# vidify/old-audiosync

Hardware: AMD Instinct MI355X
Metric: cross-correlations/sec (N=1440000 float32 pairs) (higher is better)
Workload: dtype f32; 1 GPU; batched xcorr, N=1440000 frames/sample (source 2N), 124 pairs per GPU per step, 48 kHz mono float32, planted delays, SNR 0 dB; sample_len=1440000, pairs_per_gpu=124, group=124, split=600x2400x16, layout=real-column, parallelism=pairs sharded over 1 GPU(s), one process per GPU, RCCL all_gather of results

## Files before the change

include/audiosync/xcorr_hip.h:

```cpp
#ifndef AUDIOSYNC_XCORR_HIP_H
#define AUDIOSYNC_XCORR_HIP_H

#include <stddef.h>
#include <stdint.h>

#ifdef __cplusplus
extern "C" {
#endif

typedef struct asx_plan asx_plan;


int asx_device_count(void);
int asx_current_device(void);
const char *asx_last_error(void);
int asx_abi_version(void);


asx_plan *asx_plan_create(size_t sample_len, size_t max_batch, int device);
asx_plan *asx_plan_create_ex(size_t sample_len, size_t max_batch, int device, const char *split);
int asx_plan_placement(asx_plan *plan, double ms[2], int *kept);
void asx_plan_destroy(asx_plan *plan);

int asx_plan_peak_overflows(asx_plan *plan, uint64_t *count);
int asx_plan_peak_repairs(asx_plan *plan, uint64_t *count);
int asx_plan_set_exact(asx_plan *plan, int on);
size_t asx_plan_peak_capacity(const asx_plan *plan);

int asx_plan_set_lag_window(asx_plan *plan, int64_t lag_min, int64_t lag_max);
int asx_plan_lag_window(const asx_plan *plan, int64_t *lag_min, int64_t *lag_max);

int asx_plan_set_pearson(asx_plan *plan, int spectral);
int asx_plan_pearson_modes(asx_plan *plan, uint64_t counts[3]);

int asx_plan_set_prune(asx_plan *plan, int on);
int asx_plan_prune_stats(asx_plan *plan, uint64_t *tiles_transformed, uint64_t *tiles_total);

int asx_plan_set_qstore(asx_plan *plan, int mode);
int asx_plan_qstore_stats(asx_plan *plan, uint64_t out[4]);

size_t asx_plan_sample_len(const asx_plan *plan);
size_t asx_plan_fft_len(const asx_plan *plan);
int asx_plan_split(const asx_plan *plan, int *m1, int *m2, int *tile_cols);
int asx_plan_layout(const asx_plan *plan);
int asx_plan_threads(const asx_plan *plan, int *threads_cols, int *threads_rows);
size_t asx_plan_group(const asx_plan *plan);
size_t asx_plan_workspace_bytes(const asx_plan *plan);


int asx_xcorr_f64(asx_plan *plan, const double *source, const double *sample, long *lag,
                  double *coefficient);
int asx_plan_narrowed_calls(asx_plan *plan, uint64_t *count);

int asx_xcorr_batch_f32(asx_plan *plan, const float *source, const float *sample, size_t batch,
// ... 214 lines not shown
```

old-audiosync_amd/__init__.py:

```python
from .hipxcorr import (
    LIB_PATH, AsxError, Plan, Stream, abi_version, device_count, lib, pearson_f64, planmath_candidates, planmath_describe, planmath_group_form, planmath_kernel_table, planmath_kernels,
    planmath_table, planmath_twiddles, band_bins, results_to_ms_dev, synth_pairs_dev, topk_best_dev, xcorr_batch_multi,
    Comm, PinnedArray, result_bytes, shard_range, closure_args, pool_closure, pool_closure_dev, phat_topk_args, pool_phat_topk_args,
)
```

old-audiosync_amd/csrc/asx_api.hip:

```cpp
#include "audiosync/xcorr_hip.h"

#include "asx_internal.h"
#include "dev_mem.h"
#include "plan_math.h"
#include "shard_driver.h"
#include "host_narrow.h"

#include <algorithm>
#include <cassert>
#include <cmath>
#include <cstdarg>
#include <cstdio>
#include <cstdlib>
#include <cstring>
#include <dlfcn.h>
#include <mutex>
#include <string>
#include <thread>
#include <type_traits>
#include <vector>

static thread_local std::string g_err;

static int fail(const char *fmt, ...)
// ... 112 lines not shown
    uint32_t *over_list = nullptr, *over_n = nullptr;
    volatile uint32_t *h_over_n = nullptr;
    size_t over_cap = 0;
    std::vector<uint32_t> h_over;
    unsigned long long repaired = 0;
    bool exact = true;
    int64_t win_lo = 0, win_hi = 0;
    bool spectral = false;
    unsigned long long *mode_count = nullptr;
    bool prunable = false;
    bool prune = false;
    unsigned long long *prune_stats = nullptr;
    int qstore = 1;
    unsigned long long *qstore_stats = nullptr;
    uint64_t qstore_redone = 0;
    bool tune_placement = false, placement_done = false;
    double placement_ms[2] = { 0.0, 0.0 };
    int placement_kept = -1;
    struct Staging {
        float *src = nullptr, *smp = nullptr;
        int64_t *lag = nullptr; double *coef = nullptr; int32_t *ret = nullptr;
    } st;
    struct Staging64 { double *src = nullptr, *smp = nullptr; } st64;
    float *pin32 = nullptr;
    unsigned long long narrowed = 0;

    bool profiling = false;
    size_t prof_depth = 1, prof_calls = 0, prof_ring = 0;
    std::vector<std::vector<hipEvent_t>> evr;
    std::vector<size_t> prof_groups;
// ... 135 lines not shown
        *p->h_over_n = 0;
        HIP_TRY(hipHostGetDevicePointer(&dptr, h, 0));
        d_over_host = (uint32_t *)dptr;
    }
    for (int l = 0; l < p->nlanes; l++) {
        p->lanes[l].pk.over_list = p->over_list;
        p->lanes[l].pk.over_n = p->over_n;
        p->lanes[l].pk.over_host = d_over_host;
        p->lanes[l].pk.over_cap = (uint32_t)p->over_cap;
    }
    p->spectral = d.rlayout != 0;
    if (const char *e = getenv("ASX_PEARSON")) p->spectral = p->spectral && strcmp(e, "direct") != 0;
    p->prune = p->prunable;
    if (const char *e = getenv("ASX_PRUNE")) p->prune = p->prune && atoi(e) != 0;
    if (const char *e = getenv("ASX_QSTORE")) p->qstore = std::min(2, std::max(0, atoi(e)));
    if (const char *e = getenv("ASX_EXACT")) p->exact = atoi(e) != 0;
    p->win_lo = -(int64_t)p->host.N;
    p->win_hi = (int64_t)p->host.N - 1;
    HIP_TRY(hipEventCreateWithFlags(&p->fork, hipEventDisableTiming));
    d.stamps = nullptr;
    d.stamp_kernel = 0;
    if (const char *e = getenv("ASX_STAMPS")) {
        unsigned long long *st = nullptr;
        p->stamp_blocks = g * (size_t)std::max(h.M1 + 1, 2 * h.ntiles);
        if (dev_alloc(m, &st, p->stamp_blocks * 8)) return -1;
        HIP_TRY(hipMemset(st, 0, p->stamp_blocks * 8 * sizeof(unsigned long long)));
        d.stamps = st;
        d.stamp_kernel = !strcmp(e, "fwd") ? 1 : !strcmp(e, "inv") ? 2 : 0;
    }
    {
// ... 205 lines not shown
    HIP_TRY(hipMemcpy(v, p->prune_stats, sizeof v, hipMemcpyDeviceToHost));
    *tiles_transformed = v[0];
    *tiles_total = v[1];
    return 0;
}

extern "C" int asx_plan_set_qstore(asx_plan *p, int mode)
{
    if (!p) return fail("asx_plan_set_qstore: null argument");
    if (mode < 0 || mode > 2) return fail("asx_plan_set_qstore: mode %d (0 off, 1 auto, 2 always)", mode);
    std::lock_guard<std::mutex> guard(p->lock);
    p->qstore = mode;
    return 0;
}

extern "C" int asx_plan_qstore_stats(asx_plan *p, uint64_t out[4])
{
    if (!p || !out) return fail("asx_plan_qstore_stats: null argument");
    PlanCall c(p);
    if (!c.dg.ok) return fail("cannot select device %d", p->device);
    out[0] = out[1] = out[2] = out[3] = 0;
    if (!p->qstore_stats) return 0;
    HIP_TRY(hipDeviceSynchronize());
    unsigned long long v[4];
    HIP_TRY(hipMemcpy(v, p->qstore_stats, sizeof v, hipMemcpyDeviceToHost));
    out[0] = v[0]; out[1] = v[1]; out[2] = p->qstore_redone; out[3] = v[3];
    return 0;
}

extern "C" int asx_plan_peak_repairs(asx_plan *p, uint64_t *count)
// ... 250 lines not shown
    const AsxGroupForm form = asx_group_form(
        { .rlayout = P.rlayout != 0, .plan_prune = p->prune, .plan_spectral = p->spectral, .band_sums = pk.band != nullptr,
          .over_list = pk.over_list != nullptr, .f32_inputs = std::is_same<TIn, float>::value, .f32_abi = o.f32_abi, .listed = o.listed,
          .r_out = o.r_out != nullptr, .own_lists = o.pk != nullptr, .k = o.topk.k, .search = call.kind, .weight = o.weight,
          .pool = x.pool != nullptr, .bc = x.bc, .qstore = o.qstore });
    const AsxPeakWs fin = form.appends ? pk : asx_peak_unlisted(pk);
    const AsxPeakWs tk = form.tail == ASX_TAIL_SPECTRAL ? pk : asx_peak_unbanded(pk);
    const AsxPoolPair *pl = x.pool ? W.pool : nullptr;
    const AsxSpectra &from = pl ? p->bank.c : p->bslot;
    const AsxSpectra C{ (pl || (x.bc & 1)) ? from.cx : W.zxa, (pl || (x.bc & 2)) ? from.cy : W.zya, pk.nrm_part, tk.band, form.bc, pl };
    AsxPrune U = W.prune;
    U.q_rows = form.qstore ? asx_qstore_rows(P, (int)g, p->qstore) : 0;
    U.q_row_a = P.M1 / 3;
    U.pair_base = o.pair_base;
    if (!U.q_rows) { U.list = nullptr; U.redo = nullptr; }
    if (mark(0)) return -1;
    if (form.fwd == ASX_FWD_POOL) {
        const AsxPoolArgs A{ x.pool->rows, (uint64_t)x.first, (uint64_t)x.pool->nsrc, (uint64_t)x.pool->nsmp, (uint64_t)x.src_step,
                             (uint64_t)x.smp_step, from.nrm, from.band };
        asx_launch_pool_resolve(P, A, W.pool, C.nrm, C.band, (int)g, s);
    } else if (form.fwd == ASX_FWD_REAL) {
        asx_launch_fwd_cols_r(P, (x.bc & 1) ? nullptr : x.src, x.src_step, (x.bc & 2) ? nullptr : x.smp, x.smp_step, 0, (int)g, C, false, s);
        for (unsigned which = 0; which < 2; which++)
            if (x.bc & (1 << which)) asx_launch_bcast_aux(P, from.nrm, from.band, C.nrm, C.band, (int)g, which, s);
    } else if (x.src_step == 2 * (size_t)P.N && x.smp_step == P.N) {
        asx_launch_fwd_cols(P, x.src, x.smp, W.zxa, W.zya, tk, (int)g, s);
    } else {
        for (size_t k = 0; k < g; k++) {
            AsxPeakWs one = tk;
            one.nrm_part = pk.nrm_part + k * 2 * (size_t)P.ntiles;
// ... 12 lines not shown
    auto search = [&](int j) { return AsxSearch::of(p->win_lo, p->win_hi, P.N, x.win, x.win_step, W.tk, j); };
    const double votes = form.weight == ASX_W_PHAT_BAND ? o.fband.votes(P.N) : (double)P.F;
    auto pass = [&](const AsxSearch &find, bool first) -> int {
        float *const r_out = first ? o.r_out : nullptr;
        if (form.rows == ASX_ROWS_PACKED) asx_launch_inv_cols(P, q, tk, r_out, (int)g, s, find);
        else asx_launch_inv_cols_r(P, q, tk, r_out, (int)g, s, find, form.pruned ? &U : nullptr);
        if (first && mark(3)) return -1;
        if (form.tail == ASX_TAIL_PHAT) {
            asx_launch_phat_finalize(P, fin, W.seg, K > 1 ? nullptr : y.peak, votes, (int)g, s, find);
            if (first && mark(4)) return -1;
            asx_launch_pearson(in, P.N, W.seg, W.psums, out.lag, out.coef, out.ret, (int)g, s);
            if (o.near.frac)
                asx_launch_phat_near(P, q, W.seg, votes, o.near.h, find, pl, o.near.frac, o.near.near, (int)g, s);
            return 0;
        }
        asx_launch_finalize(P, fin, W.seg, (int)g, s, o.pair_base, find);
        asx_launch_refine(P, in, pk, W.seg, (int)g, s, dot_blocks, form.tail == ASX_TAIL_DIRECT, find);
        if (first && mark(4)) return -1;
        if (form.tail == ASX_TAIL_DIRECT)
            asx_launch_pearson(in, P.N, W.seg, W.psums, out.lag, out.coef, out.ret, (int)g, s);
        else if constexpr (std::is_same<TIn, float>::value)
            asx_launch_pearson_spectral_f32(P, in, find, tk, W.spec, W.seg, W.psums, out.lag, out.coef, out.ret, (int)g, s);
        return 0;
    };
    if (pass(call, true)) return -1;
    if (U.q_rows && form.takeback) asx_launch_qstore_takeback(U, W.spec, (int)g, s);
    if (call.kind == AsxSearch::ROWS && K == 1) asx_launch_invalid_rows(call.rows, P.N, y.lag, y.coef, y.ret, (int)g, s);
    if (pl && K == 1) asx_launch_invalid_pairs(pl, y.lag, y.coef, y.ret, y.peak, (int)g, s);
    for (int j = 0; K > 1 && j < K; j++) {
        if (j > 0 && pass(search(j), false)) return -1;
        if (form.tail == ASX_TAIL_PHAT && y.peak) asx_launch_topk_peak(W.tk, pk, call, P.N, (int)g, j, K, votes, y.peak, s);
        asx_launch_topk_step(W.tk, W.seg, pk, call, P.N, (int)g, j, K, o.topk.sep, y.lag, y.coef, y.ret, s);
    }
    if (pl && K > 1) asx_launch_invalid_pairs_k(pl, K, y.lag, y.coef, y.ret, y.peak, (int)g, s);
    if (mark(5)) return -1;
    HIP_TRY(hipGetLastError());
    return 0;
}

template <typename TIn>
static int second_look(asx_plan *p, const Pairs<TIn> &xi, const Results &yi, hipStream_t s, const Topk &topk)
// ... 1392 lines not shown

extern "C" int asx_planmath_group_form(const int *ask, int nask, int *out, int nout)
{
    if (!ask || !out || nask != ASX_GROUP_ASK_INTS || nout != ASX_GROUP_FORM_INTS)
        return fail("asx_planmath_group_form: %d and %d ints, not %d and %d", nask, nout, ASX_GROUP_ASK_INTS, ASX_GROUP_FORM_INTS);
    AsxGroupAsk a;
    a.rlayout = ask[0]; a.plan_prune = ask[1]; a.plan_spectral = ask[2]; a.band_sums = ask[3]; a.over_list = ask[4];
    a.f32_inputs = ask[5]; a.f32_abi = ask[6]; a.listed = ask[7]; a.r_out = ask[8]; a.own_lists = ask[9]; a.k = ask[10];
    a.search = ask[11]; a.weight = (AsxWeight)ask[12]; a.pool = ask[13]; a.bc = ask[14]; a.qstore = ask[15];
    const AsxGroupForm f = asx_group_form(a);
    const int v[ASX_GROUP_FORM_INTS] = { f.fwd, f.rows, f.weight, f.bc, f.pruned, f.tail, f.appends, f.qstore, f.takeback };
    memcpy(out, v, sizeof v);
    return 0;
}

extern "C" int asx_planmath_describe(size_t sample_len, const char *split, uint32_t *F, uint32_t *src_valid,
                                     int *M1, int *M2, int *T, int *nst1, int *radix1, int *nst2,
                                     int *radix2)
{
    AsxHostPlan h;
    std::string err = asx_host_plan_build(sample_len, split, &h);
    if (!err.empty()) return fail("%s", err.c_str());
    *F = h.F; *src_valid = h.src_valid; *M1 = h.M1; *M2 = h.M2; *T = h.T;
    *nst1 = h.st1.nstages; *nst2 = h.st2.nstages;
    for (int i = 0; i < h.st1.nstages; i++) radix1[i] = h.st1.radix[i];
    for (int i = 0; i < h.st2.nstages; i++) radix2[i] = h.st2.radix[i];
    return 0;
}

extern "C" int asx_planmath_candidates(size_t sample_len, size_t max_count, char *out, size_t cap)
// ... 32 lines not shown
```

old-audiosync_amd/csrc/asx_internal.h:

```cpp
#pragma once

#include <hip/hip_runtime.h>
#include <stdint.h>
#include <type_traits>

#define ASX_MAX_STAGES 12
#define ASX_TW_LOG 11
#define ASX_TW_LO (1u << ASX_TW_LOG)
#define ASX_THREADS 256
#define ASX_FFT_THREADS_MAX 512
#define ASX_COL_LOADS 10
#define ASX_ROW_STEPS 5
#define ASX_PEARSON_BLOCKS_MAX 512
#define ASX_DC_STATS_DOUBLES (4 + 2 * 128)
#define ASX_BOUND_C 4.0f
#define ASX_PRUNE_DELTA 6.103515625e-5f
#define ASX_PRUNE_FLOOR_PER_TERM 3.944304526105059e-31
#define ASX_PRUNE_T 16
#define ASX_Q_ALL 0xFFFFFFFFFFFFFFFFull
#define ASX_QSTORE_C 1.75
#define ASX_QSTORE_REDO 0x80000000u
__host__ __device__ inline bool asx_q_stored(unsigned long long w, int tile)
{
    const unsigned t = (unsigned)tile;
// ... 422 lines not shown
void asx_launch_pool_resolve(const AsxDev &P, const AsxPoolArgs &A, AsxPoolPair *out, float *nrm, float2 *band, int npairs,
                             hipStream_t s);
void asx_launch_invalid_pairs(const AsxPoolPair *pl, int64_t *lag, double *coef, int32_t *ret, double *peak, int npairs, hipStream_t s);
void asx_launch_invalid_pairs_k(const AsxPoolPair *pl, int k, int64_t *lag, double *coef, int32_t *ret, double *peak, int npairs,
                                hipStream_t s);
void asx_launch_finalize(const AsxDev &P, const AsxPeakWs &W, AsxSeg *seg, int npairs, hipStream_t s, uint32_t pair_base,
                         const AsxSearch &q);
void asx_launch_topk_step(AsxTopkWs T, const AsxSeg *seg, const AsxPeakWs &W, const AsxSearch &call, uint32_t N, int npairs, int j,
                          int k, int64_t sep, int64_t *lag, double *coef, int32_t *ret, hipStream_t s);
void asx_launch_topk_peak(const AsxTopkWs &T, const AsxPeakWs &W, const AsxSearch &call, uint32_t N, int npairs, int j, int k, double f,
                          double *peak, hipStream_t s);
void asx_launch_invalid_rows(const AsxWinRows &rows, uint32_t N, int64_t *lag, double *coef, int32_t *ret, int npairs, hipStream_t s);
template <typename TIn>
void asx_launch_refine(const AsxDev &P, const AsxInputs<TIn> &in, const AsxPeakWs &W, AsxSeg *seg, int npairs, hipStream_t s,
                       int dot_blocks, bool pick, const AsxSearch &q);
template <typename TIn>
void asx_launch_pearson(const AsxInputs<TIn> &in, uint32_t basis_len, const AsxSeg *seg, double *psums, int64_t *lag, double *coef,
                        int32_t *ret, int npairs, hipStream_t s);
void asx_launch_pearson_partial_spec_f32(const AsxInputs<float> &in, uint32_t basis_len, const AsxSeg *seg, const AsxSpecWs &S,
                                         double *psums, int npairs, hipStream_t s);
void asx_launch_pearson_spectral_f32(const AsxDev &P, const AsxInputs<float> &in, const AsxSearch &q, const AsxPeakWs &W,
                                     const AsxSpecWs &S, AsxSeg *seg, double *psums, int64_t *lag, double *coef, int32_t *ret,
                                     int npairs, hipStream_t s);
int asx_launch_debug_spec_pick(const AsxDev &P, const AsxSpecWs &S, const AsxSeg *seg, size_t pair, double *out, hipStream_t s);
void asx_launch_results_to_ms(const int64_t *lag, const double *coef, const int32_t *ret, size_t batch,
                              double min_confidence, double sample_rate, int64_t *lag_ms, int32_t *accept,
                              hipStream_t s);
void asx_launch_topk_best(const int64_t *lag, const double *coef, const int32_t *ret, size_t batch, int k, int64_t *best_lag,
                          double *best_coef, int32_t *best_ret, int32_t *best_entry, hipStream_t s);
#define ASX_CLOSURE_LAG_LIMIT ((int64_t)1 << 40)
void asx_launch_pool_closure(const int64_t *lag, const double *coef, const int32_t *ret, uint32_t C, int k, int64_t tol,
                             int min_confirm, int root, int32_t *votes, int64_t *best_lag, double *best_coef, int32_t *best_ret,
                             int32_t *best_entry, int32_t *confirm, int32_t *d_root, int64_t *offset, int32_t *support,
                             int32_t *placed, hipStream_t s);
void asx_launch_cvt_f64_f32(const double *in, float *out, size_t n, hipStream_t s);
unsigned asx_pearson_blocks(uint32_t basis_len);
template <typename TIn>
void asx_launch_dc_remove(const TIn *src, const TIn *smp, uint32_t N, double scale, double *stats, float *out, hipStream_t s);
// ... 3 lines not shown
```

old-audiosync_amd/csrc/pearson_spectral.hip:

```cpp
#include "asx_internal.h"
#include "xcorr_dev.h"


static_assert(ASX_PREP_BLOCKS <= ASX_PREP_BLOCKS_MAX, "AsxSpecWs::part is sized for ASX_PREP_BLOCKS_MAX blocks per pair");
#ifndef ASX_PREP_THREADS
#define ASX_PREP_THREADS 1024
#endif

namespace {

struct Acc2 {
    double s1, s2;
};

__device__ __forceinline__ void acc1(Acc2 &a, float f)
{
    const double v = (double)f;
    a.s1 += v;
    a.s2 = fma(v, v, a.s2);
}
__device__ __forceinline__ void acc4(Acc2 &a, float4 v) { acc1(a, v.x); acc1(a, v.y); acc1(a, v.z); acc1(a, v.w); }

template <uint32_t NTP> __device__ __forceinline__ void direct_range(const float *__restrict__ x, uint32_t lo, uint32_t hi, Acc2 &a, uint32_t tid)
{
// ... 120 lines not shown
template <int NTP, int NB> __global__ __launch_bounds__(NTP) void k_pearson_prep_xl(const AsxDev *__restrict__ Pp, const float *__restrict__ src,
                                                                       const float *__restrict__ smp, const AsxPoolPair *__restrict__ PL,
                                                                       AsxPeakWs W, AsxSpecWs S, AsxSeg *__restrict__ seg,
                                                                       const AsxTopkPair *__restrict__ X)
{
    const uint32_t seed = X[blockIdx.y].z.seed;
#define ASX_SRC_OF(pair) PL[pair].src_off
#define ASX_SMP_OF(pair) PL[pair].smp_off
#include "pearson_prep_body.h"
}

__global__ __launch_bounds__(64) void k_pearson_final_spec(const AsxSeg *__restrict__ seg, const double *__restrict__ psums, uint32_t nb,
                                                            AsxSpecWs S, int64_t *__restrict__ lag,
                                                            double *__restrict__ coef, int32_t *__restrict__ ret)
{
    const size_t pair = blockIdx.x;
    const AsxSeg s = seg[pair];
    const AsxSpecPick d = asx_spec_pick(s, S.part + pair * (size_t)(S.nb * 4), S.nb, S.hdr + pair * ASX_SPEC_HDR, S.tol, S.N);
    const int mode = (int)S.hdr[pair * ASX_SPEC_HDR + 3];
    PStat v;
    v.n = v.mx = v.my = v.mxx = v.myy = v.cxy = 0.0;
    if (mode != ASX_PM_FAST) {
        for (uint32_t b = threadIdx.x; b < nb; b += 64u) {
            const double *p = psums + (pair * nb + b) * 6;
            PStat o;
            o.n = p[0];
            if (o.n != 0.0) { o.mx = p[1]; o.my = p[2]; o.mxx = p[3]; o.myy = p[4]; o.cxy = p[5]; v = pstat_merge(v, o); }
        }
        v = pstat_wave_merge(v);
    }
    if (threadIdx.x == 0) {
        double c;
        if (mode == ASX_PM_DIRECT) {
            c = v.cxy / sqrt(v.mxx * v.myy);
        } else {
            const double n = d.n, Sx = d.Sx, Sxx = d.Sxx, Sy = d.Sy, Syy = d.Syy;
            double sxy = d.r;
            if (mode == ASX_PM_CORR) sxy -= v.cxy + v.n * v.mx * v.my;
            c = (sxy - Sx * Sy / n) / sqrt((Sxx - Sx * Sx / n) * (Syy - Sy * Sy / n));
            c = c > 1.0 ? 1.0 : c < -1.0 ? -1.0 : c;
        }
        if (lag) lag[pair] = s.lag;
        coef[pair] = c;
        if (ret) ret[pair] = (s.flags & ASX_SEG_INEXACT) ? 1 : (c != c) ? -1 : 0;
        atomicAdd(S.mode_count + mode, 1ull);
    }
}

template <int NTP, int NB>
static void launch_prep(const AsxDev &P, const AsxInputs<float> &in, const AsxSearch &q, const AsxPeakWs &W, const AsxSpecWs &S,
                        AsxSeg *seg, int npairs, hipStream_t s)
{
    const dim3 grid(NB, npairs), block(NTP);
    if (in.pl && q.kind == AsxSearch::TOPK)
        hipLaunchKernelGGL((k_pearson_prep_xl<NTP, NB>), grid, block, 0, s, P.self_dev, in.src, in.smp, in.pl, W, S, seg, q.tk);
    else if (in.pl && q.kind == AsxSearch::ROWS)
        hipLaunchKernelGGL((k_pearson_prep_pl<NTP, NB>), grid, block, 0, s, P.self_dev, in.src, in.smp, in.pl, W, S, seg, q.rows);
    else if (in.pl)
        hipLaunchKernelGGL((k_pearson_prep_l<NTP, NB>), grid, block, 0, s, P.self_dev, in.src, in.smp, in.pl, W, S, seg, q.seed());
    else if (q.kind == AsxSearch::TOPK)
        hipLaunchKernelGGL((k_pearson_prep_x<NTP, NB>), grid, block, 0, s, P.self_dev, in.src, in.smp, in.src_pitch, in.smp_pitch, W, S,
                           seg, q.tk);
    else if (q.kind == AsxSearch::ROWS)
        hipLaunchKernelGGL((k_pearson_prep_p<NTP, NB>), grid, block, 0, s, P.self_dev, in.src, in.smp, in.src_pitch, in.smp_pitch, W, S,
                           seg, q.rows);
    else
        hipLaunchKernelGGL((k_pearson_prep<NTP, NB>), grid, block, 0, s, P.self_dev, in.src, in.smp, in.src_pitch, in.smp_pitch, W, S,
                           seg, q.seed());
}

static bool prep_long_tracks(const AsxDev &P) { return (size_t)P.band_rows * (size_t)P.M2 >= 16384; }

void asx_launch_pearson_spectral_f32(const AsxDev &P, const AsxInputs<float> &in, const AsxSearch &q, const AsxPeakWs &W,
                                     const AsxSpecWs &S0, AsxSeg *seg, double *psums, int64_t *lag, double *coef, int32_t *ret,
                                     int npairs, hipStream_t s)
{
    AsxSpecWs S = S0;
    S.N = P.N;
    const bool long_tracks = prep_long_tracks(P);
    S.nb = long_tracks ? ASX_PREP_BLOCKS : 1;
    if (long_tracks) launch_prep<ASX_PREP_THREADS, ASX_PREP_BLOCKS>(P, in, q, W, S, seg, npairs, s);
    else launch_prep<256, 1>(P, in, q, W, S, seg, npairs, s);
    asx_launch_pearson_partial_spec_f32(in, P.N, seg, S, psums, npairs, s);
    hipLaunchKernelGGL(k_pearson_final_spec, dim3(npairs), dim3(64), 0, s, seg, psums, asx_pearson_blocks(P.N), S, lag, coef, ret);
}

__global__ __launch_bounds__(64) void k_debug_spec_pick(const AsxSeg *__restrict__ seg, AsxSpecWs S, size_t pair, double *__restrict__ out)
{
    if (threadIdx.x != 0 || blockIdx.x != 0) return;
    const AsxSpecPick d = asx_spec_pick(seg[pair], S.part + pair * (size_t)(S.nb * 4), S.nb, S.hdr + pair * ASX_SPEC_HDR, S.tol, S.N);
    out[0] = (double)d.mode; out[1] = d.n; out[2] = d.Sx; out[3] = d.Sxx; out[4] = d.Sy; out[5] = d.Syy; out[6] = d.r; out[7] = d.bound;
}

int asx_launch_debug_spec_pick(const AsxDev &P, const AsxSpecWs &S0, const AsxSeg *seg, size_t pair, double *out, hipStream_t s)
{
    AsxSpecWs S = S0;
    S.N = P.N;
    S.nb = prep_long_tracks(P) ? ASX_PREP_BLOCKS : 1;
    hipLaunchKernelGGL(k_debug_spec_pick, dim3(1), dim3(1), 0, s, seg, S, pair, out);
// ... 3 lines not shown
```

old-audiosync_amd/csrc/plan_math.cpp:

```cpp
#include <cstring>
#include <cstdlib>
#include <functional>
#include <algorithm>
#include "plan_math.h"
#include "kernel_table.h"

#include <cmath>
#include <cstdio>
#include <cstdlib>

bool asx_is_smooth(uint64_t n)
{
    if (n == 0) return false;
    for (uint64_t p : { 2ull, 3ull, 5ull })
        while (n % p == 0) n /= p;
    return n == 1;
}

uint64_t asx_next_smooth_even(uint64_t n)
{
    n += n & 1ull;
    if (n < 2) n = 2;
    while (!asx_is_smooth(n)) n += 2;
    return n;
// ... 309 lines not shown
    AsxGroupForm f{};
    f.weight = a.weight;
    f.bc = a.bc;
    const bool phat = a.weight != ASX_W_NONE;
    f.appends = a.listed && !phat;
    const bool spectral = a.f32_inputs && a.plan_spectral && a.f32_abi && a.band_sums && !phat;
    f.tail = phat ? ASX_TAIL_PHAT : spectral ? ASX_TAIL_SPECTRAL : ASX_TAIL_DIRECT;
    f.pruned = a.plan_prune && !phat && a.f32_inputs && a.f32_abi && !a.pool && a.bc == 0 && !a.r_out && !a.own_lists && a.k == 1 &&
               a.search == AsxSearch::ALL;
    f.qstore = f.pruned && a.listed && a.qstore && a.over_list;
    f.takeback = f.qstore && spectral;
    f.fwd = a.pool ? ASX_FWD_POOL : a.rlayout ? ASX_FWD_REAL : ASX_FWD_PACKED;
    f.rows = !a.rlayout ? ASX_ROWS_PACKED : f.pruned ? ASX_ROWS_ENERGY : a.pool ? ASX_ROWS_LISTED : ASX_ROWS_PLAIN;
    return f;
}
```

old-audiosync_amd/csrc/plan_math.h:

```cpp
#pragma once

#include "asx_internal.h"

#include <string>
#include <vector>

struct AsxKernelChoice {
    bool rlayout = false;
    int cols = -1, rows = -1;
    int threads_cols = 0, threads_rows = 0;
    int band_rows = 0;
    bool prunable = false;
};

struct AsxHostPlan {
    size_t N = 0;
    uint32_t F = 0, M = 0, src_valid = 0;
    int M1 = 0, M2 = 0, T = 0, logT = 0, ntiles = 0;
    AsxStages st1{}, st2{};
    std::vector<float2> tw1, tw2, tw2s, tw_lo, tw_hi;
    std::vector<int> k1_of_pos1, pos1_of_k1, pos2_of_k2;
    std::vector<int4> row_tasks;
    bool rlayout = false;
    std::vector<int4> col_pairs;
// ... 34 lines not shown
};
enum AsxFwdForm { ASX_FWD_POOL, ASX_FWD_REAL, ASX_FWD_PACKED };
enum AsxTail { ASX_TAIL_PHAT, ASX_TAIL_DIRECT, ASX_TAIL_SPECTRAL };
struct AsxGroupForm {
    AsxFwdForm fwd;
    AsxRowFlavour rows;
    AsxWeight weight;
    int bc;
    bool pruned;
    AsxTail tail;
    bool appends;
    bool qstore;
    bool takeback;
};
AsxGroupForm asx_group_form(const AsxGroupAsk &a);
constexpr int ASX_GROUP_ASK_INTS = 16, ASX_GROUP_FORM_INTS = 9;
```

old-audiosync_amd/csrc/xcorr_kernels.hip:

```cpp
#include "asx_internal.h"
#include "lds_fft.h"
#include "xcorr_dev.h"
#include "kernel_table.h"

#include <algorithm>
#include <math.h>
#include <type_traits>
#include <stdlib.h>

#ifndef ASX_PART
#define ASX_PART 127
#endif
#define ASX_HAS_PART(bit) ((ASX_PART & (bit)) != 0)

#ifdef ASX_STAMPS
#define ASX_STAMP_AT(kernel, block, slot)                                                            \
    do {                                                                                             \
        if (P.stamps && P.stamp_kernel == (kernel) && threadIdx.x == 0)                              \
            P.stamps[(size_t)(block) * 8 + (slot)] = clock64();                                      \
    } while (0)
#else
#define ASX_STAMP_AT(kernel, block, slot) do {} while (0)
#endif
#define ASX_STAMP(slot) ASX_STAMP_AT(0, task, slot)
// ... 970 lines not shown
        __syncthreads();
        if (threadIdx.x == 0) {
            dd_t t;
            t.hi = red[0][0]; t.lo = red[1][0];
            for (int w = 1; w < ASX_THREADS / 64; w++) {
                dd_t o;
                o.hi = red[0][w]; o.lo = red[1][w];
                t = dd_add(t, o);
            }
            W.refine_val[pair * (size_t)W.cap + c] = t.hi + t.lo;
        }
        __syncthreads();
    }
}

template <class Sel>
__global__ __launch_bounds__(ASX_THREADS) void k_refine_pick(const AsxDev *__restrict__ Pp, AsxPeakWs W, AsxSeg *__restrict__ seg,
                                                              Sel sel)
{
    const uint32_t seed = sel.seed_of(blockIdx.x, Pp->N);
    __shared__ double rkey[ASX_THREADS / 64];
    __shared__ uint32_t ridx[ASX_THREADS / 64];
    const size_t pair = blockIdx.x;
    const uint32_t n = W.refine_n[pair];
    if (n < 2u) return;
    double bk = -INFINITY;
    uint32_t bi = 0xFFFFFFFFu;
    for (uint32_t i = threadIdx.x; i < n; i += ASX_THREADS) {
        const uint32_t idx = W.refine_idx[pair * (size_t)W.cap + i];
        const double v = W.refine_val[pair * (size_t)W.cap + i];
// ... 1238 lines not shown
template <typename TIn>
void asx_launch_refine(const AsxDev &P, const AsxInputs<TIn> &in, const AsxPeakWs &W, AsxSeg *seg, int npairs, hipStream_t s,
                       int dot_blocks, bool pick, const AsxSearch &q)
{
    asx_with_inputs(in, [&](auto at) {
        hipLaunchKernelGGL((k_refine_dots<TIn, decltype(at)>), dim3(dot_blocks, npairs), dim3(ASX_THREADS), 0, s, P.self_dev, in.src,
                           in.smp, at, W);
    });
    if (!pick) return;
    const dim3 grid(npairs), block(ASX_THREADS);
    asx_with_selection(q, [&](auto sel) {
        hipLaunchKernelGGL(k_refine_pick<decltype(sel)>, grid, block, 0, s, P.self_dev, W, seg, sel);
    });
}

unsigned asx_pearson_blocks(uint32_t basis_len)
{
    const uint32_t per_block = 16u * 4u * ASX_THREADS;
    uint32_t nb = (basis_len + per_block - 1) / per_block;
    if (nb > ASX_PEARSON_BLOCKS_MAX) nb = ASX_PEARSON_BLOCKS_MAX;
    if (nb < 1) nb = 1;
    return nb;
}

template <typename TIn, bool SPEC>
static void launch_pearson_partial(const AsxInputs<TIn> &in, uint32_t basis_len, const AsxSeg *seg, const AsxSpecWs &S, double *psums,
                                   int npairs, hipStream_t s)
{
    const dim3 grid(asx_pearson_blocks(basis_len), npairs), block(ASX_THREADS);
    asx_with_inputs(in, [&](auto at) {
// ... 169 lines not shown
```

old-audiosync_amd/hipxcorr.py:

```python
import ctypes
import os
import sys

import numpy as np

_HERE = os.path.dirname(os.path.abspath(__file__))
LIB_PATH = os.path.join(_HERE, "libaudiosync_hip.so")
_lib = None

c_f32p = ctypes.POINTER(ctypes.c_float)
c_f64p = ctypes.POINTER(ctypes.c_double)
c_i64p = ctypes.POINTER(ctypes.c_int64)
c_i32p = ctypes.POINTER(ctypes.c_int32)
c_intp = ctypes.POINTER(ctypes.c_int)

_vp, _sz, _int, _i64, _u64, _dbl, _str = (ctypes.c_void_p, ctypes.c_size_t, ctypes.c_int, ctypes.c_int64, ctypes.c_uint64,
                                          ctypes.c_double, ctypes.c_char_p)
_vpp, _szp, _longp = ctypes.POINTER(_vp), ctypes.POINTER(_sz), ctypes.POINTER(ctypes.c_long)
_u32p, _u64p = ctypes.POINTER(ctypes.c_uint32), ctypes.POINTER(ctypes.c_uint64)

_HEADER_SIGNATURES = {
    "asx_device_count": (_int, []),
    "asx_current_device": (_int, []),
    "asx_last_error": (_str, []),
# ... 11 lines not shown
    "asx_plan_layout": (_int, [_vp]),
    "asx_plan_peak_overflows": (_int, [_vp, _u64p]),
    "asx_plan_peak_repairs": (_int, [_vp, _u64p]),
    "asx_plan_narrowed_calls": (_int, [_vp, _u64p]),
    "asx_plan_set_exact": (_int, [_vp, _int]),
    "asx_plan_set_lag_window": (_int, [_vp, _i64, _i64]),
    "asx_plan_lag_window": (_int, [_vp, c_i64p, c_i64p]),
    "asx_stream_set_lag_window": (_int, [_vp, _i64, _i64]),
    "asx_plan_placement": (_int, [_vp, c_f64p, c_intp]),
    "asx_plan_set_pearson": (_int, [_vp, _int]),
    "asx_plan_pearson_modes": (_int, [_vp, _u64p]),
    "asx_plan_set_prune": (_int, [_vp, _int]),
    "asx_plan_prune_stats": (_int, [_vp, _u64p, _u64p]),
    "asx_plan_set_qstore": (_int, [_vp, _int]),
    "asx_plan_qstore_stats": (_int, [_vp, _u64p]),
    "asx_plan_set_profiling": (_int, [_vp, _int]),
    "asx_plan_last_timings_ms": (_int, [_vp, c_f32p]),
    "asx_plan_timings_ms": (_int, [_vp, _int, c_f32p]),
    "asx_xcorr_f64": (_int, [_vp, c_f64p, c_f64p, _longp, c_f64p]),
    "asx_xcorr_batch_f32": (_int, [_vp, c_f32p, c_f32p, _sz, c_i64p, c_f64p, c_i32p]),
    "asx_xcorr_batch_multi": (_int, [_vpp, _int, c_f32p, c_f32p, _sz, c_i64p, c_f64p, c_i32p]),
    "asx_xcorr_batch_f32_dev": (_int, [_vp, _vp, _vp, _sz, _vp, _vp, _vp, _vp]),
    "asx_xcorr_strided_f32_dev": (_int, [_vp, _vp, _sz, _vp, _sz, _sz, _vp, _vp, _vp, _vp]),
    "asx_xcorr_windowed_f32_dev": (_int, [_vp, _vp, _sz, _vp, _sz, _vp, _sz, _sz, _vp, _vp, _vp, _vp]),
    "asx_xcorr_topk_f32_dev": (_int, [_vp, _vp, _sz, _vp, _sz, _vp, _sz, _sz, _int, _i64, _vp, _vp, _vp, _vp]),
    "asx_xcorr_phat_f32_dev": (_int, [_vp, _vp, _sz, _vp, _sz, _vp, _sz, _sz, _vp, _vp, _vp, _vp, _vp]),
    "asx_xcorr_phat_band_f32_dev": (_int, [_vp, _vp, _sz, _vp, _sz, _vp, _sz, _sz, _i64, _i64, _vp, _vp, _vp, _vp, _vp]),
    "asx_xcorr_phat_sub_f32_dev": (_int, [_vp, _vp, _sz, _vp, _sz, _vp, _sz, _sz, _i64, _i64, _int, _vp, _vp, _vp, _vp, _vp, _vp, _vp]),
    "asx_xcorr_phat_topk_f32_dev": (_int, [_vp, _vp, _sz, _vp, _sz, _vp, _sz, _sz, _i64, _i64, _int, _i64, _vp, _vp, _vp, _vp, _vp]),
    "asx_xcorr_pool_f32_dev": (_int, [_vp, _vp, _sz, _sz, _vp, _sz, _sz, _vp, _vp, _sz, _sz, _vp, _vp, _vp, _vp]),
# ... 36 lines not shown
    "asx_host_malloc": (_vp, [_sz]),
    "asx_host_free": (_int, [_vp]),
    "asx_memcpy_h2d": (_int, [_vp, _vp, _sz]),
    "asx_memcpy_d2h": (_int, [_vp, _vp, _sz]),
    "asx_stream_sync": (_int, [_vp, _vp]),
}

_DIAGNOSTIC_SIGNATURES = {
    "asx_planmath_describe": (_int, [_sz, _str, _u32p, _u32p, c_intp, c_intp, c_intp, c_intp, c_intp, c_intp, c_intp]),
    "asx_planmath_table": (_int, [_sz, _str, _int, c_intp, _sz]),
    "asx_planmath_twiddles": (_int, [_sz, _str, _int, c_f32p, _sz]),
    "asx_planmath_candidates": (_int, [_sz, _sz, _str, _sz]),
    "asx_planmath_kernels": (_int, [_sz, _str, c_intp, c_intp, c_intp]),
    "asx_planmath_kernel_table": (_int, [_int, _int, c_intp]),
    "asx_planmath_group_form": (_int, [c_intp, _int, c_intp, _int]),
    "asx_plan_debug_kernels": (_int, [_vp, c_intp, c_intp, c_intp]),
    "asx_plan_debug_bank": (_int, [_vp, _u64p, _u64p, _u64p]),
    "asx_plan_debug_prune": (_int, [_vp, _sz, c_f32p, c_intp, _sz]),
    "asx_plan_debug_peak": (_int, [_vp, _sz, c_f32p, _u32p, _u32p, _u64p, _vp, _vp, _sz]),
    "asx_plan_debug_spectral": (_int, [_vp, _sz, c_intp, _vp, _sz, c_f64p, ctypes.POINTER(ctypes.c_longlong), c_f64p]),
    "asx_plan_debug_over_list": (_int, [_vp, _u32p, _u32p]),
    "asx_plan_debug_stamps": (ctypes.c_long, [_vp, _vp, _sz]),
}

SIGNATURES = {**_HEADER_SIGNATURES, **_DIAGNOSTIC_SIGNATURES}

ABI_SYMBOLS = list(_HEADER_SIGNATURES)

TOPK_MAX = 8
NEAR_MAX = 8
# ... 114 lines not shown
GROUP_ASK = ("rlayout", "plan_prune", "plan_spectral", "band_sums", "over_list", "f32_inputs", "f32_abi", "listed", "r_out",
             "own_lists", "k", "search", "weight", "pool", "bc", "qstore")
GROUP_FORM = ("fwd", "rows", "weight", "bc", "pruned", "tail", "appends", "qstore", "takeback")
GROUP_ENUMS = {"search": ("all", "window", "rows", "topk"), "weight": ("none", "phat", "phat-band"),
               "fwd": ("pool", "real-column", "packed"), "rows": ("packed", "plain", "energy", "listed"),
               "tail": ("phat", "direct", "spectral")}


def planmath_group_form(**ask):
    if set(ask) != set(GROUP_ASK):
        raise ValueError("planmath_group_form: the ask is %s" % (GROUP_ASK,))
    a = (ctypes.c_int * len(GROUP_ASK))(*(GROUP_ENUMS[n].index(ask[n]) if n in GROUP_ENUMS else int(ask[n]) for n in GROUP_ASK))
    out = (ctypes.c_int * len(GROUP_FORM))()
    _check(lib().asx_planmath_group_form(a, len(a), out, len(out)))
    return {n: GROUP_ENUMS[n][v] if n in GROUP_ENUMS else v if n == "bc" else bool(v) for n, v in zip(GROUP_FORM, out)}


def planmath_candidates(sample_len, max_count=16):
    buf = ctypes.create_string_buffer(64 * max_count + 1)
    n = lib().asx_planmath_candidates(sample_len, max_count, buf, len(buf))
    if n < 0:
        raise AsxError(_err())
    return [x for x in buf.value.decode().split("\n") if x]


def planmath_table(sample_len, which, split=None):
    d = planmath_describe(sample_len, split)
    cap = max(d["M1"], d["M2"])
    buf = (ctypes.c_int * cap)()
    n = lib().asx_planmath_table(sample_len, _split_arg(split), which, buf, cap)
# ... 526 lines not shown

    def pearson_modes(self):
        c = (ctypes.c_uint64 * 3)()
        _check(lib().asx_plan_pearson_modes(self._h, c))
        return tuple(int(v) for v in c)

    def set_prune(self, on=True):
        _check(lib().asx_plan_set_prune(self._h, 1 if on else 0))

    def prune_stats(self):
        return _counters(lib().asx_plan_prune_stats, self._h, 2)

    def set_qstore(self, mode=1):
        _check(lib().asx_plan_set_qstore(self._h, int(mode)))

    def qstore_stats(self):
        c = (ctypes.c_uint64 * 4)()
        _check(lib().asx_plan_qstore_stats(self._h, c))
        return tuple(int(v) for v in c)

    def narrowed_calls(self):
        return _counters(lib().asx_plan_narrowed_calls, self._h, 1)[0]

    def peak_repairs(self):
        return _counters(lib().asx_plan_peak_repairs, self._h, 1)[0]

    @property
    def workspace_bytes(self):
        return lib().asx_plan_workspace_bytes(self._h)

# ... 412 lines not shown
```

Before: 63380 cross-correlations/s.

## Fuse finalize with refine dot products and skip qstore takeback pass

```diff
diff --git a/include/audiosync/xcorr_hip.h b/include/audiosync/xcorr_hip.h
--- a/include/audiosync/xcorr_hip.h
+++ b/include/audiosync/xcorr_hip.h
@@ -38,6 +38,8 @@
 
 int asx_plan_set_qstore(asx_plan *plan, int mode);
 int asx_plan_qstore_stats(asx_plan *plan, uint64_t out[4]);
+
+int asx_plan_set_tail(asx_plan *plan, int on);
 
 size_t asx_plan_sample_len(const asx_plan *plan);
 size_t asx_plan_fft_len(const asx_plan *plan);
diff --git a/old-audiosync_amd/__init__.py b/old-audiosync_amd/__init__.py
--- a/old-audiosync_amd/__init__.py
+++ b/old-audiosync_amd/__init__.py
@@ -1,5 +1,5 @@
 from .hipxcorr import (
-    LIB_PATH, AsxError, Plan, Stream, abi_version, device_count, lib, pearson_f64, planmath_candidates, planmath_describe, planmath_group_form, planmath_kernel_table, planmath_kernels,
+    LIB_PATH, AsxError, Plan, Stream, abi_version, device_count, lib, pearson_f64, planmath_candidates, planmath_describe, planmath_group_form, planmath_group_tail, planmath_kernel_table, planmath_kernels,
     planmath_table, planmath_twiddles, band_bins, results_to_ms_dev, synth_pairs_dev, topk_best_dev, xcorr_batch_multi,
     Comm, PinnedArray, result_bytes, shard_range, closure_args, pool_closure, pool_closure_dev, phat_topk_args, pool_phat_topk_args,
 )
diff --git a/old-audiosync_amd/csrc/asx_api.hip b/old-audiosync_amd/csrc/asx_api.hip
--- a/old-audiosync_amd/csrc/asx_api.hip
+++ b/old-audiosync_amd/csrc/asx_api.hip
@@ -150,6 +150,7 @@
     int qstore = 1;
     unsigned long long *qstore_stats = nullptr;
     uint64_t qstore_redone = 0;
+    bool tail = true;
     bool tune_placement = false, placement_done = false;
     double placement_ms[2] = { 0.0, 0.0 };
     int placement_kept = -1;
@@ -315,6 +316,7 @@
     p->prune = p->prunable;
     if (const char *e = getenv("ASX_PRUNE")) p->prune = p->prune && atoi(e) != 0;
     if (const char *e = getenv("ASX_QSTORE")) p->qstore = std::min(2, std::max(0, atoi(e)));
+    if (const char *e = getenv("ASX_TAIL")) p->tail = atoi(e) != 0;
     if (const char *e = getenv("ASX_EXACT")) p->exact = atoi(e) != 0;
     p->win_lo = -(int64_t)p->host.N;
     p->win_hi = (int64_t)p->host.N - 1;
@@ -550,6 +552,14 @@
     return 0;
 }
 
+extern "C" int asx_plan_set_tail(asx_plan *p, int on)
+{
+    if (!p) return fail("asx_plan_set_tail: null argument");
+    std::lock_guard<std::mutex> guard(p->lock);
+    p->tail = on != 0;
+    return 0;
+}
+
 extern "C" int asx_plan_qstore_stats(asx_plan *p, uint64_t out[4])
 {
     if (!p || !out) return fail("asx_plan_qstore_stats: null argument");
@@ -830,6 +840,7 @@
     U.q_row_a = P.M1 / 3;
     U.pair_base = o.pair_base;
     if (!U.q_rows) { U.list = nullptr; U.redo = nullptr; }
+    const bool short_tail = asx_group_tail_short(form, U.q_rows, p->tail);
     if (mark(0)) return -1;
     if (form.fwd == ASX_FWD_POOL) {
         const AsxPoolArgs A{ x.pool->rows, (uint64_t)x.first, (uint64_t)x.pool->nsrc, (uint64_t)x.pool->nsmp, (uint64_t)x.src_step,
@@ -872,17 +883,23 @@
                 asx_launch_phat_near(P, q, W.seg, votes, o.near.h, find, pl, o.near.frac, o.near.near, (int)g, s);
             return 0;
         }
-        asx_launch_finalize(P, fin, W.seg, (int)g, s, o.pair_base, find);
-        asx_launch_refine(P, in, pk, W.seg, (int)g, s, dot_blocks, form.tail == ASX_TAIL_DIRECT, find);
+        bool fused = false;
+        if constexpr (std::is_same<TIn, float>::value)
+            fused = short_tail && asx_launch_finalize_dots_f32(P, in, fin, W.seg, (int)g, s, dot_blocks, o.pair_base, find);
+        if (!fused) {
+            asx_launch_finalize(P, fin, W.seg, (int)g, s, o.pair_base, find);
+            asx_launch_refine(P, in, pk, W.seg, (int)g, s, dot_blocks, form.tail == ASX_TAIL_DIRECT, find);
+        }
         if (first && mark(4)) return -1;
         if (form.tail == ASX_TAIL_DIRECT)
             asx_launch_pearson(in, P.N, W.seg, W.psums, out.lag, out.coef, out.ret, (int)g, s);
         else if constexpr (std::is_same<TIn, float>::value)
-            asx_launch_pearson_spectral_f32(P, in, find, tk, W.spec, W.seg, W.psums, out.lag, out.coef, out.ret, (int)g, s);
+            asx_launch_pearson_spectral_f32(P, in, find, tk, W.spec, W.seg, W.psums, out.lag, out.coef, out.ret, (int)g, s,
+                                            short_tail ? U.redo : nullptr);
         return 0;
     };
     if (pass(call, true)) return -1;
-    if (U.q_rows && form.takeback) asx_launch_qstore_takeback(U, W.spec, (int)g, s);
+    if (U.q_rows && form.takeback && !short_tail) asx_launch_qstore_takeback(U, W.spec, (int)g, s);
     if (call.kind == AsxSearch::ROWS && K == 1) asx_launch_invalid_rows(call.rows, P.N, y.lag, y.coef, y.ret, (int)g, s);
     if (pl && K == 1) asx_launch_invalid_pairs(pl, y.lag, y.coef, y.ret, y.peak, (int)g, s);
     for (int j = 0; K > 1 && j < K; j++) {
@@ -2305,6 +2322,15 @@
     return 0;
 }
 
+extern "C" int asx_planmath_group_tail(const int *ask, int nask, int q_rows, int plan_tail)
+{
+    int form[ASX_GROUP_FORM_INTS];
+    if (asx_planmath_group_form(ask, nask, form, ASX_GROUP_FORM_INTS)) return -1;
+    AsxGroupForm f{};
+    f.qstore = form[7]; f.takeback = form[8];
+    return asx_group_tail_short(f, q_rows, plan_tail != 0) ? 1 : 0;
+}
+
 extern "C" int asx_planmath_describe(size_t sample_len, const char *split, uint32_t *F, uint32_t *src_valid,
                                      int *M1, int *M2, int *T, int *nst1, int *radix1, int *nst2,
                                      int *radix2)
diff --git a/old-audiosync_amd/csrc/asx_internal.h b/old-audiosync_amd/csrc/asx_internal.h
--- a/old-audiosync_amd/csrc/asx_internal.h
+++ b/old-audiosync_amd/csrc/asx_internal.h
@@ -460,6 +460,8 @@
 template <typename TIn>
 void asx_launch_refine(const AsxDev &P, const AsxInputs<TIn> &in, const AsxPeakWs &W, AsxSeg *seg, int npairs, hipStream_t s,
                        int dot_blocks, bool pick, const AsxSearch &q);
+bool asx_launch_finalize_dots_f32(const AsxDev &P, const AsxInputs<float> &in, const AsxPeakWs &W, AsxSeg *seg, int npairs, hipStream_t s,
+                                  int dot_blocks, uint32_t pair_base, const AsxSearch &q);
 template <typename TIn>
 void asx_launch_pearson(const AsxInputs<TIn> &in, uint32_t basis_len, const AsxSeg *seg, double *psums, int64_t *lag, double *coef,
                         int32_t *ret, int npairs, hipStream_t s);
@@ -467,7 +469,7 @@
                                          double *psums, int npairs, hipStream_t s);
 void asx_launch_pearson_spectral_f32(const AsxDev &P, const AsxInputs<float> &in, const AsxSearch &q, const AsxPeakWs &W,
                                      const AsxSpecWs &S, AsxSeg *seg, double *psums, int64_t *lag, double *coef, int32_t *ret,
-                                     int npairs, hipStream_t s);
+                                     int npairs, hipStream_t s, const unsigned char *voided = nullptr);
 int asx_launch_debug_spec_pick(const AsxDev &P, const AsxSpecWs &S, const AsxSeg *seg, size_t pair, double *out, hipStream_t s);
 void asx_launch_results_to_ms(const int64_t *lag, const double *coef, const int32_t *ret, size_t batch,
                               double min_confidence, double sample_rate, int64_t *lag_ms, int32_t *accept,
diff --git a/old-audiosync_amd/csrc/pearson_final_body.h b/old-audiosync_amd/csrc/pearson_final_body.h
--- /dev/null
+++ b/old-audiosync_amd/csrc/pearson_final_body.h
@@ -0,0 +1,31 @@
+    const size_t pair = blockIdx.x;
+    const AsxSeg s = seg[pair];
+    const AsxSpecPick d = asx_spec_pick(s, S.part + pair * (size_t)(S.nb * 4), S.nb, S.hdr + pair * ASX_SPEC_HDR, S.tol, S.N);
+    const int mode = (int)S.hdr[pair * ASX_SPEC_HDR + 3];
+    PStat v;
+    v.n = v.mx = v.my = v.mxx = v.myy = v.cxy = 0.0;
+    if (mode != ASX_PM_FAST) {
+        for (uint32_t b = threadIdx.x; b < nb; b += 64u) {
+            const double *p = psums + (pair * nb + b) * 6;
+            PStat o;
+            o.n = p[0];
+            if (o.n != 0.0) { o.mx = p[1]; o.my = p[2]; o.mxx = p[3]; o.myy = p[4]; o.cxy = p[5]; v = pstat_merge(v, o); }
+        }
+        v = pstat_wave_merge(v);
+    }
+    if (threadIdx.x == 0) {
+        double c;
+        if (mode == ASX_PM_DIRECT) {
+            c = v.cxy / sqrt(v.mxx * v.myy);
+        } else {
+            const double n = d.n, Sx = d.Sx, Sxx = d.Sxx, Sy = d.Sy, Syy = d.Syy;
+            double sxy = d.r;
+            if (mode == ASX_PM_CORR) sxy -= v.cxy + v.n * v.mx * v.my;
+            c = (sxy - Sx * Sy / n) / sqrt((Sxx - Sx * Sx / n) * (Syy - Sy * Sy / n));
+            c = c > 1.0 ? 1.0 : c < -1.0 ? -1.0 : c;
+        }
+        if (lag) lag[pair] = s.lag;
+        coef[pair] = c;
+        if (ret) ret[pair] = (s.flags & ASX_SEG_INEXACT) ? 1 : (c != c) ? -1 : 0;
+        if (counted) atomicAdd(S.mode_count + mode, 1ull);
+    }
diff --git a/old-audiosync_amd/csrc/pearson_spectral.hip b/old-audiosync_amd/csrc/pearson_spectral.hip
--- a/old-audiosync_amd/csrc/pearson_spectral.hip
+++ b/old-audiosync_amd/csrc/pearson_spectral.hip
@@ -158,37 +158,16 @@
                                                             AsxSpecWs S, int64_t *__restrict__ lag,
                                                             double *__restrict__ coef, int32_t *__restrict__ ret)
 {
-    const size_t pair = blockIdx.x;
-    const AsxSeg s = seg[pair];
-    const AsxSpecPick d = asx_spec_pick(s, S.part + pair * (size_t)(S.nb * 4), S.nb, S.hdr + pair * ASX_SPEC_HDR, S.tol, S.N);
-    const int mode = (int)S.hdr[pair * ASX_SPEC_HDR + 3];
-    PStat v;
-    v.n = v.mx = v.my = v.mxx = v.myy = v.cxy = 0.0;
-    if (mode != ASX_PM_FAST) {
-        for (uint32_t b = threadIdx.x; b < nb; b += 64u) {
-            const double *p = psums + (pair * nb + b) * 6;
-            PStat o;
-            o.n = p[0];
-            if (o.n != 0.0) { o.mx = p[1]; o.my = p[2]; o.mxx = p[3]; o.myy = p[4]; o.cxy = p[5]; v = pstat_merge(v, o); }
-        }
-        v = pstat_wave_merge(v);
-    }
-    if (threadIdx.x == 0) {
-        double c;
-        if (mode == ASX_PM_DIRECT) {
-            c = v.cxy / sqrt(v.mxx * v.myy);
-        } else {
-            const double n = d.n, Sx = d.Sx, Sxx = d.Sxx, Sy = d.Sy, Syy = d.Syy;
-            double sxy = d.r;
-            if (mode == ASX_PM_CORR) sxy -= v.cxy + v.n * v.mx * v.my;
-            c = (sxy - Sx * Sy / n) / sqrt((Sxx - Sx * Sx / n) * (Syy - Sy * Sy / n));
-            c = c > 1.0 ? 1.0 : c < -1.0 ? -1.0 : c;
-        }
-        if (lag) lag[pair] = s.lag;
-        coef[pair] = c;
-        if (ret) ret[pair] = (s.flags & ASX_SEG_INEXACT) ? 1 : (c != c) ? -1 : 0;
-        atomicAdd(S.mode_count + mode, 1ull);
-    }
+    constexpr bool counted = true;
+#include "pearson_final_body.h"
+}
+
+__global__ __launch_bounds__(64) void k_pearson_final_spec_v(const AsxSeg *__restrict__ seg, const double *__restrict__ psums, uint32_t nb,
+                                                              AsxSpecWs S, int64_t *__restrict__ lag, double *__restrict__ coef,
+                                                              int32_t *__restrict__ ret, const unsigned char *__restrict__ redo)
+{
+    const bool counted = !redo[blockIdx.x];
+#include "pearson_final_body.h"
 }
 
 template <int NTP, int NB>
@@ -217,7 +196,7 @@
 
 void asx_launch_pearson_spectral_f32(const AsxDev &P, const AsxInputs<float> &in, const AsxSearch &q, const AsxPeakWs &W,
                                      const AsxSpecWs &S0, AsxSeg *seg, double *psums, int64_t *lag, double *coef, int32_t *ret,
-                                     int npairs, hipStream_t s)
+                                     int npairs, hipStream_t s, const unsigned char *voided)
 {
     AsxSpecWs S = S0;
     S.N = P.N;
@@ -226,7 +205,10 @@
     if (long_tracks) launch_prep<ASX_PREP_THREADS, ASX_PREP_BLOCKS>(P, in, q, W, S, seg, npairs, s);
     else launch_prep<256, 1>(P, in, q, W, S, seg, npairs, s);
     asx_launch_pearson_partial_spec_f32(in, P.N, seg, S, psums, npairs, s);
-    hipLaunchKernelGGL(k_pearson_final_spec, dim3(npairs), dim3(64), 0, s, seg, psums, asx_pearson_blocks(P.N), S, lag, coef, ret);
+    if (voided)
+        hipLaunchKernelGGL(k_pearson_final_spec_v, dim3(npairs), dim3(64), 0, s, seg, psums, asx_pearson_blocks(P.N), S, lag, coef, ret, voided);
+    else
+        hipLaunchKernelGGL(k_pearson_final_spec, dim3(npairs), dim3(64), 0, s, seg, psums, asx_pearson_blocks(P.N), S, lag, coef, ret);
 }
 
 __global__ __launch_bounds__(64) void k_debug_spec_pick(const AsxSeg *__restrict__ seg, AsxSpecWs S, size_t pair, double *__restrict__ out)
diff --git a/old-audiosync_amd/csrc/plan_math.cpp b/old-audiosync_amd/csrc/plan_math.cpp
--- a/old-audiosync_amd/csrc/plan_math.cpp
+++ b/old-audiosync_amd/csrc/plan_math.cpp
@@ -347,3 +347,8 @@
     f.rows = !a.rlayout ? ASX_ROWS_PACKED : f.pruned ? ASX_ROWS_ENERGY : a.pool ? ASX_ROWS_LISTED : ASX_ROWS_PLAIN;
     return f;
 }
+
+bool asx_group_tail_short(const AsxGroupForm &f, int q_rows, bool plan_tail)
+{
+    return plan_tail && f.qstore && f.takeback && q_rows > 0;
+}
diff --git a/old-audiosync_amd/csrc/plan_math.h b/old-audiosync_amd/csrc/plan_math.h
--- a/old-audiosync_amd/csrc/plan_math.h
+++ b/old-audiosync_amd/csrc/plan_math.h
@@ -72,4 +72,5 @@
     bool takeback;
 };
 AsxGroupForm asx_group_form(const AsxGroupAsk &a);
+bool asx_group_tail_short(const AsxGroupForm &f, int q_rows, bool plan_tail);
 constexpr int ASX_GROUP_ASK_INTS = 16, ASX_GROUP_FORM_INTS = 9;
diff --git a/old-audiosync_amd/csrc/xcorr_kernels.hip b/old-audiosync_amd/csrc/xcorr_kernels.hip
--- a/old-audiosync_amd/csrc/xcorr_kernels.hip
+++ b/old-audiosync_amd/csrc/xcorr_kernels.hip
@@ -1008,6 +1008,118 @@
     }
 }
 
+template <typename TIn>
+__device__ __forceinline__ void refine_dot(const TIn *__restrict__ x, const TIn *__restrict__ y, uint32_t N, uint32_t k,
+                                           double (*red)[ASX_THREADS / 64], double *__restrict__ dst)
+{
+    const uint32_t L = 2u * N;
+    const int lane = threadIdx.x & 63, wave = threadIdx.x >> 6;
+    double hi = 0.0, lo = 0.0;
+    for (uint32_t n = threadIdx.x; n < N; n += ASX_THREADS) {
+        uint32_t i = n + k;
+        if (i >= L) i -= L;
+        const double a = (double)x[i], b = (double)y[n];
+        const double p = a * b;
+        double pe = 0.0;
+        if (sizeof(TIn) == sizeof(double)) pe = fma(a, b, -p);
+        const double s = hi + p;
+        const double bb = s - hi;
+        lo += ((hi - (s - bb)) + (p - bb)) + pe;
+        hi = s;
+    }
+    dd_t acc;
+    acc.hi = hi; acc.lo = lo;
+#pragma unroll
+    for (int off = 32; off > 0; off >>= 1) {
+        dd_t o;
+        o.hi = __shfl_xor(acc.hi, off, 64);
+        o.lo = __shfl_xor(acc.lo, off, 64);
+        acc = dd_add(acc, o);
+    }
+    if (lane == 0) { red[0][wave] = acc.hi; red[1][wave] = acc.lo; }
+    __syncthreads();
+    if (threadIdx.x == 0) {
+        dd_t t;
+        t.hi = red[0][0]; t.lo = red[1][0];
+        for (int w = 1; w < ASX_THREADS / 64; w++) {
+            dd_t o;
+            o.hi = red[0][w]; o.lo = red[1][w];
+            t = dd_add(t, o);
+        }
+        *dst = t.hi + t.lo;
+    }
+    __syncthreads();
+}
+
+constexpr int FD_OWN = ASX_CAND_MAX / 8;
+template <typename TIn, class Where>
+__global__ __launch_bounds__(ASX_THREADS) void k_finalize_dots(const AsxDev *__restrict__ Pp, const TIn *__restrict__ src,
+                                                                const TIn *__restrict__ smp, Where at, AsxPeakWs W,
+                                                                AsxSeg *__restrict__ seg, uint32_t pair_base, uint32_t seed)
+{
+    __shared__ double red[2][ASX_THREADS / 64];
+    __shared__ uint32_t own[FD_OWN];
+    __shared__ uint32_t wcount[ASX_THREADS / 64];
+    const size_t pair = blockIdx.x;
+    const uint32_t bx = blockIdx.y, nbx = gridDim.y;
+    const bool writer = bx == 0;
+    const uint32_t ntot = W.cand_n[pair];
+    if (!writer && bx >= ntot) return;
+    const uint32_t N = Pp->N;
+    const int lane = threadIdx.x & 63, wave = threadIdx.x >> 6;
+    const asx_peak_t best = W.pairmax[pair];
+    const bool over = ntot > W.cap;
+    const uint32_t n = (over || ntot < 2u) ? 0u : ntot;
+    uint32_t nsel = 0;
+    if (n) {
+        const float thr = near_max_threshold(peak_key(best), W.bound2[pair]);
+        const AsxCand *c = W.cand + pair * (size_t)W.cap;
+        uint32_t *out = W.refine_idx + pair * (size_t)W.cap;
+        for (uint32_t i0 = 0; i0 < n; i0 += ASX_THREADS) {
+            const uint32_t i = i0 + threadIdx.x;
+            AsxCand e{ 0u, 0.f };
+            if (i < n) e = c[i];
+            const bool keep = i < n && e.key >= thr;
+            const unsigned long long m = __ballot(keep);
+            if (lane == 0) wcount[wave] = (uint32_t)__popcll(m);
+            __syncthreads();
+            uint32_t at_c = nsel + (uint32_t)__popcll(m & ((1ull << lane) - 1ull)), all = 0;
+            for (int w = 0; w < ASX_THREADS / 64; w++) {
+                at_c += w < wave ? wcount[w] : 0u;
+                all += wcount[w];
+            }
+            if (keep) {
+                if (writer) out[at_c] = e.idx;
+                if (at_c % nbx == bx) own[at_c / nbx] = e.idx;
+            }
+            nsel += all;
+            __syncthreads();
+        }
+    }
+    const uint32_t ncand = nsel >= 2u ? nsel : 0u;
+    if (writer && threadIdx.x == 0) {
+        AsxSeg sg = make_seg(best ? peak_index(best) : seed, N);
+        if (over) sg.flags = ASX_SEG_INEXACT;
+        seg[pair] = sg;
+        W.refine_n[pair] = ncand;
+        if (over) {
+            atomicAdd(W.overflows, 1ull);
+            if (W.over_list) {
+                const uint32_t slot = atomicAdd(W.over_n, 1u);
+                if (slot < W.over_cap) W.over_list[slot] = pair_base + (uint32_t)pair;
+                if (W.over_host) (void)__hip_atomic_fetch_add(W.over_host, 1u, __ATOMIC_RELAXED, __HIP_MEMORY_SCOPE_SYSTEM);
+            }
+        }
+    }
+    if (bx >= ncand) return;
+    const TIn *x = src + at.src_off(pair);
+    const TIn *y = smp + at.smp_off(pair);
+    for (uint32_t c = bx; c < ncand; c += nbx) {
+        const uint32_t k = own[c / nbx];
+        refine_dot(x, y, N, k, red, W.refine_val + pair * (size_t)W.cap + c);
+    }
+}
+
 template <class Sel>
 __global__ __launch_bounds__(ASX_THREADS) void k_refine_pick(const AsxDev *__restrict__ Pp, AsxPeakWs W, AsxSeg *__restrict__ seg,
                                                               Sel sel)
@@ -2276,6 +2388,17 @@
     });
 }
 
+bool asx_launch_finalize_dots_f32(const AsxDev &P, const AsxInputs<float> &in, const AsxPeakWs &W, AsxSeg *seg, int npairs, hipStream_t s,
+                                  int dot_blocks, uint32_t pair_base, const AsxSearch &q)
+{
+    if (in.pl || (q.kind != AsxSearch::ALL && q.kind != AsxSearch::WINDOW) || dot_blocks < 1 ||
+        (size_t)W.cap > (size_t)FD_OWN * (size_t)dot_blocks)
+        return false;
+    hipLaunchKernelGGL((k_finalize_dots<float, AsxAtPitch>), dim3(npairs, dot_blocks), dim3(ASX_THREADS), 0, s, P.self_dev, in.src, in.smp,
+                       AsxAtPitch{ in.src_pitch, in.smp_pitch }, W, seg, pair_base, q.seed());
+    return true;
+}
+
 unsigned asx_pearson_blocks(uint32_t basis_len)
 {
     const uint32_t per_block = 16u * 4u * ASX_THREADS;
diff --git a/old-audiosync_amd/hipxcorr.py b/old-audiosync_amd/hipxcorr.py
--- a/old-audiosync_amd/hipxcorr.py
+++ b/old-audiosync_amd/hipxcorr.py
@@ -49,6 +49,7 @@
     "asx_plan_prune_stats": (_int, [_vp, _u64p, _u64p]),
     "asx_plan_set_qstore": (_int, [_vp, _int]),
     "asx_plan_qstore_stats": (_int, [_vp, _u64p]),
+    "asx_plan_set_tail": (_int, [_vp, _int]),
     "asx_plan_set_profiling": (_int, [_vp, _int]),
     "asx_plan_last_timings_ms": (_int, [_vp, c_f32p]),
     "asx_plan_timings_ms": (_int, [_vp, _int, c_f32p]),
@@ -115,6 +116,7 @@
     "asx_planmath_kernels": (_int, [_sz, _str, c_intp, c_intp, c_intp]),
     "asx_planmath_kernel_table": (_int, [_int, _int, c_intp]),
     "asx_planmath_group_form": (_int, [c_intp, _int, c_intp, _int]),
+    "asx_planmath_group_tail": (_int, [c_intp, _int, _int, _int]),
     "asx_plan_debug_kernels": (_int, [_vp, c_intp, c_intp, c_intp]),
     "asx_plan_debug_bank": (_int, [_vp, _u64p, _u64p, _u64p]),
     "asx_plan_debug_prune": (_int, [_vp, _sz, c_f32p, c_intp, _sz]),
@@ -259,6 +261,16 @@
     out = (ctypes.c_int * len(GROUP_FORM))()
     _check(lib().asx_planmath_group_form(a, len(a), out, len(out)))
     return {n: GROUP_ENUMS[n][v] if n in GROUP_ENUMS else v if n == "bc" else bool(v) for n, v in zip(GROUP_FORM, out)}
+
+
+def planmath_group_tail(q_rows, plan_tail=True, **ask):
+    if set(ask) != set(GROUP_ASK):
+        raise ValueError("planmath_group_tail: the ask is %s" % (GROUP_ASK,))
+    a = (ctypes.c_int * len(GROUP_ASK))(*(GROUP_ENUMS[n].index(ask[n]) if n in GROUP_ENUMS else int(ask[n]) for n in GROUP_ASK))
+    v = lib().asx_planmath_group_tail(a, len(a), int(q_rows), 1 if plan_tail else 0)
+    if v < 0:
+        raise AsxError(_err())
+    return bool(v)
 
 
 def planmath_candidates(sample_len, max_count=16):
@@ -815,6 +827,9 @@
     def set_qstore(self, mode=1):
         _check(lib().asx_plan_set_qstore(self._h, int(mode)))
 
+    def set_tail(self, on=True):
+        _check(lib().asx_plan_set_tail(self._h, 1 if on else 0))
+
     def qstore_stats(self):
         c = (ctypes.c_uint64 * 4)()
         _check(lib().asx_plan_qstore_stats(self._h, c))
```

Result: no change. 63360 cross-correlations/s (-0.0%).
